# hideki1217/rusTfhe

Measured on AMD Instinct MI355X. Metric: HomNAND gates/sec (whole node), N=1024, higher is better.
Workload: dtype f64

## Files before the change

rustfhe_amd/csrc/rtfhe_context.hip:

```cpp
#include "rtfhe_host.hpp"

#include <cmath>
#include <cstdio>
#include <cstdlib>
#include <map>
#include <mutex>

using namespace rtfhe;
using namespace rtfhe_host;

namespace {

thread_local std::string g_last_error;

std::mutex g_lds_mutex;
std::map<std::pair<int, const void*>, size_t> g_lds_granted;

int ensure_pinned(rtfhe_ctx* ctx, int slot, size_t bytes) {
    if (ctx->cap_pin[slot] >= bytes && ctx->h_pin[slot]) return 0;
    if (ctx->h_pin[slot]) HIPCHECK(ctx, hipHostFree(ctx->h_pin[slot]));
    ctx->h_pin[slot] = nullptr; ctx->cap_pin[slot] = 0;
    HIPCHECK(ctx, hipHostMalloc(&ctx->h_pin[slot], bytes ? bytes : 16, hipHostMallocDefault));
    ctx->cap_pin[slot] = bytes;
    return 0;
// ... 303 lines not shown
    if (ctx->d_a) (void)hipFree(ctx->d_a);
    if (ctx->d_b) (void)hipFree(ctx->d_b);
    if (ctx->d_c) (void)hipFree(ctx->d_c);
    for (void* h : ctx->h_pin) if (h) (void)hipHostFree(h);
    for (auto& kv : ctx->mux) for (void* m : kv.second.m) if (m) (void)hipFree(m);
    for (void* m : ctx->mux_retired) (void)hipFree(m);
    for (hipEvent_t e : ctx->ks_events) (void)hipEventDestroy(e);
    if (ctx->ev0) (void)hipEventDestroy(ctx->ev0);
    if (ctx->ev1) (void)hipEventDestroy(ctx->ev1);
    if (ctx->ev_shard) (void)hipEventDestroy(ctx->ev_shard);
    for (hipEvent_t e : ctx->ev_sh) if (e) (void)hipEventDestroy(e);
    if (ctx->stream) (void)hipStreamDestroy(ctx->stream);
    delete ctx;
}

int rtfhe_set_backend(rtfhe_ctx* ctx, int backend) {
    if (int rc = use(ctx)) return rc;
    if (backend != RTFHE_BACKEND_FFT64_MIRROR && backend != RTFHE_BACKEND_NTT_EXACT && backend != RTFHE_BACKEND_FFT_SPLIT_EXACT)
        return fail(ctx, RTFHE_ERR_INVALID, "unknown backend");
    ctx->backend = backend;
    for (rtfhe_ctx* peer : ctx->peers) peer->backend = backend;
    return 0;
}

int rtfhe_get_backend(const rtfhe_ctx* ctx) { return ctx ? ctx->backend : RTFHE_ERR_INVALID; }

int rtfhe_ctx_params(const rtfhe_ctx* ctx, rtfhe_params* p) {
    if (!ctx || !p) return fail(nullptr, RTFHE_ERR_INVALID, "null argument");
    *p = ctx->p;
    return 0;
}

int rtfhe_get_twiddles(const rtfhe_ctx* ctx, double* ifft_table, double* fft_table) {
    if (!ctx || !ifft_table || !fft_table) return fail(nullptr, RTFHE_ERR_INVALID, "null argument");
    ctx->tw.export_ref(ifft_table, fft_table);
    return 0;
}

int rtfhe_set_twiddles(rtfhe_ctx* ctx, const double* ifft_table, const double* fft_table) {
    if (int rc = use(ctx)) return rc;
    if (!ifft_table || !fft_table) return fail(ctx, RTFHE_ERR_INVALID, "null argument");
    const HostTw before = ctx->tw;
    ctx->tw.import_ref(ifft_table, fft_table);
    HIPCHECK(ctx, hipDeviceSynchronize());
    if (int rc = upload_twiddles(ctx)) { ctx->tw = before; return rc; }
    if (ctx->has_bk && ctx->d_bk_torus) {
        if (int rc = transform_bk_from_torus(ctx)) return rc;
        key_changed(ctx);
        if (int rc = rebuild_derived_keys(ctx)) return rc;
    }
    for (rtfhe_ctx* peer : ctx->peers) {
        if (int rc = rtfhe_set_twiddles(peer, ifft_table, fft_table)) return fail(ctx, rc, peer->err);
        HIPCHECK(ctx, hipSetDevice(ctx->device));
    }
    return 0;
}

int rtfhe_twiddles_write(const rtfhe_ctx* ctx, const char* path) {
    if (!ctx || !path) return fail(nullptr, RTFHE_ERR_INVALID, "null argument");
    std::vector<double> t((size_t)4 * ctx->p.N);
    ctx->tw.export_ref(t.data(), t.data() + (size_t)2 * ctx->p.N);
    return rtfhe_twiddles_file_write(path, ctx->p.N, t.data(), t.data() + (size_t)2 * ctx->p.N);
}

int rtfhe_twiddles_load(rtfhe_ctx* ctx, const char* path, int32_t* entries_changed) {
    if (!ctx || !path) return fail(nullptr, RTFHE_ERR_INVALID, "null argument");
    if (entries_changed) *entries_changed = 0;
    const size_t n2 = (size_t)2 * ctx->p.N;
    std::vector<double> t(2 * n2), cur(2 * n2);
    if (rtfhe_twiddles_file_read(path, ctx->p.N, t.data(), t.data() + n2) != 0)
        return fail(ctx, RTFHE_ERR_INVALID, "twiddle table file: unreadable, wrong degree or checksum mismatch");
    ctx->tw.export_ref(cur.data(), cur.data() + n2);
    int32_t diff = 0;
    for (size_t i = 0; i < t.size(); i++) diff += std::memcmp(&t[i], &cur[i], sizeof(double)) != 0;
    if (entries_changed) *entries_changed = diff;
    if (diff == 0) return 0;
    return rtfhe_set_twiddles(ctx, t.data(), t.data() + n2);
}

int rtfhe_load_bk_torus(rtfhe_ctx* ctx, const uint32_t* bk) {
    if (int rc = use(ctx)) return rc;
    if (!bk) return fail(ctx, RTFHE_ERR_INVALID, "null argument");
    const size_t words = bk_word_count(ctx->p);
    if (!ctx->d_bk) HIPCHECK(ctx, hipMalloc((void**)&ctx->d_bk, bk_cplx_count(ctx->p) * sizeof(cplx)));
    if (!ctx->d_bk_torus) HIPCHECK(ctx, hipMalloc((void**)&ctx->d_bk_torus, words * 4));
    HIPCHECK(ctx, hipMemcpy(ctx->d_bk_torus, bk, words * 4, hipMemcpyHostToDevice));
    if (int rc = transform_bk_from_torus(ctx)) return rc;
    key_changed(ctx);
    ctx->has_bk = true;
    if (int rc = rebuild_derived_keys(ctx)) return rc;
    for (rtfhe_ctx* peer : ctx->peers) {
        if (int rc = replicate(ctx, peer, ctx->d_bk, (void**)&peer->d_bk, bk_cplx_count(ctx->p) * sizeof(cplx))) return rc;
        if (int rc = replicate(ctx, peer, ctx->d_bk_torus, (void**)&peer->d_bk_torus, words * 4)) return rc;
        key_changed(peer); peer->has_bk = true;
        if (int rc = rebuild_derived_keys(peer)) return fail(ctx, rc, peer->err);
    }
    HIPCHECK(ctx, hipSetDevice(ctx->device));
    return 0;
}

int rtfhe_load_bk_fft(rtfhe_ctx* ctx, const double* bk_f) {
    if (int rc = use(ctx)) return rc;
    if (!bk_f) return fail(ctx, RTFHE_ERR_INVALID, "null argument");
    const size_t words = bk_word_count(ctx->p);
    if (!ctx->d_bk) HIPCHECK(ctx, hipMalloc((void**)&ctx->d_bk, bk_cplx_count(ctx->p) * sizeof(cplx)));
    if (int rc = ensure(ctx, &ctx->d_a, &ctx->cap_a, words * 8)) return rc;
    HIPCHECK(ctx, hipMemcpy(ctx->d_a, bk_f, words * 8, hipMemcpyHostToDevice));
    const size_t polys = words / ctx->p.N;
    if (int rc = launch_bk_permute(ctx, (const double*)ctx->d_a, (double*)ctx->d_bk, polys, 0, ctx->stream)) return rc;
    HIPCHECK(ctx, hipStreamSynchronize(ctx->stream));
    if (ctx->d_bk_torus) { (void)hipFree(ctx->d_bk_torus); ctx->d_bk_torus = nullptr; }
    key_changed(ctx);
    ctx->has_bk = true;
    if (int rc = rebuild_derived_keys(ctx)) return rc;
    for (rtfhe_ctx* peer : ctx->peers) {
        if (int rc = replicate(ctx, peer, ctx->d_bk, (void**)&peer->d_bk, bk_cplx_count(ctx->p) * sizeof(cplx))) return rc;
        if (peer->d_bk_torus) { (void)hipSetDevice(peer->device); (void)hipFree(peer->d_bk_torus); peer->d_bk_torus = nullptr; (void)hipSetDevice(ctx->device); }
        key_changed(peer); peer->has_bk = true;
        if (int rc = rebuild_derived_keys(peer)) return fail(ctx, rc, peer->err);
    }
    HIPCHECK(ctx, hipSetDevice(ctx->device));
    return 0;
}

int rtfhe_export_bk_fft(rtfhe_ctx* ctx, double* bk_f) {
    if (int rc = use(ctx)) return rc;
    if (!bk_f) return fail(ctx, RTFHE_ERR_INVALID, "null argument");
    if (!ctx->has_bk) return fail(ctx, RTFHE_ERR_STATE, "bootstrapping key not loaded");
    const size_t words = bk_word_count(ctx->p);
    if (int rc = ensure(ctx, &ctx->d_a, &ctx->cap_a, words * 8)) return rc;
    const size_t polys = words / ctx->p.N;
    if (int rc = launch_bk_permute(ctx, (const double*)ctx->d_bk, (double*)ctx->d_a, polys, 1, ctx->stream)) return rc;
    HIPCHECK(ctx, hipStreamSynchronize(ctx->stream));
    HIPCHECK(ctx, hipMemcpy(bk_f, ctx->d_a, words * 8, hipMemcpyDeviceToHost));
    return 0;
}

int rtfhe_load_ksk(rtfhe_ctx* ctx, const uint32_t* ksk) {
    if (int rc = use(ctx)) return rc;
    if (!ksk) return fail(ctx, RTFHE_ERR_INVALID, "null argument");
    const size_t rows = ksk_rows(ctx->p), w = (size_t)ctx->p.n + 1, ksw = (size_t)ctx->ksw;
    std::vector<uint32_t> padded((rows + 1) * ksw, 0u);
    for (size_t r = 0; r < rows; r++) std::memcpy(padded.data() + r * ksw, ksk + r * w, w * 4);
    if (int rc = ensure(ctx, &ctx->d_a, &ctx->cap_a, padded.size() * 4)) return rc;
    HIPCHECK(ctx, hipMemcpy(ctx->d_a, padded.data(), padded.size() * 4, hipMemcpyHostToDevice));
    const size_t dev_rows = (size_t)ks_dev_rows(ctx->p.N, ctx->p.ks_t, ctx->p.ks_basebit);
    ctx->ksk_bytes = (dev_rows + 1) * ksw * 4;
    if (!ctx->d_ksk) HIPCHECK(ctx, hipMalloc((void**)&ctx->d_ksk, ctx->ksk_bytes));
    if (int rc = launch_ksk_combine(ctx, (const uint32_t*)ctx->d_a, ctx->stream)) return rc;
    HIPCHECK(ctx, hipStreamSynchronize(ctx->stream));
    size_t ksmat_bytes = 0;
    if (ctx->ks_mm_min > 0) {
        const int colgroups = (ctx->p.n + 1 + 15) / 16;
        ksmat_bytes = (size_t)colgroups * (ctx->p.N / 2) * 4 * 64 * sizeof(uint4);
        if (!ctx->d_ksmat) HIPCHECK(ctx, hipMalloc((void**)&ctx->d_ksmat, ksmat_bytes));
        ctx->ksmat_bytes = ksmat_bytes;
        if (int rc = launch_ksmat_build(ctx, (const uint32_t*)ctx->d_a, colgroups, ctx->stream)) return rc;
        HIPCHECK(ctx, hipStreamSynchronize(ctx->stream));
        if (int rc = ensure_tlwe1(ctx, ctx->tlwe1[ctx->stream], 8192)) return rc;
    }
    ctx->has_ksk = true;
    for (rtfhe_ctx* peer : ctx->peers) {
        if (int rc = replicate(ctx, peer, ctx->d_ksk, (void**)&peer->d_ksk, ctx->ksk_bytes)) return rc;
        peer->ksk_bytes = ctx->ksk_bytes;
        if (ksmat_bytes) {
            if (int rc = replicate(ctx, peer, ctx->d_ksmat, (void**)&peer->d_ksmat, ksmat_bytes)) return rc;
            peer->ksmat_bytes = ksmat_bytes;
        }
        peer->has_ksk = true;
    }
    return 0;
}

int rtfhe_load_ksk_ref(rtfhe_ctx* ctx, const uint32_t* ksk_ref) {
    if (int rc = use(ctx)) return rc;
    if (!ksk_ref) return fail(ctx, RTFHE_ERR_INVALID, "null argument");
    const size_t w = (size_t)ctx->p.n + 1, base = (size_t)1 << ctx->p.ks_basebit, levels = (size_t)ctx->p.N * ctx->p.ks_t;
    std::vector<uint32_t> compact;
    try { compact.resize(levels * (base - 1) * w); } catch (const std::bad_alloc&) { return fail(ctx, RTFHE_ERR_NOMEM, "host staging for the key-switching key"); }
    for (size_t il = 0; il < levels; il++)
        std::memcpy(compact.data() + il * (base - 1) * w, ksk_ref + il * base * w, (base - 1) * w * sizeof(uint32_t));
    return rtfhe_load_ksk(ctx, compact.data());
}

}
```

rustfhe_amd/csrc/rtfhe_kernels_ksmm.hpp:

```cpp
#pragma once

#include "rtfhe_kernels.hpp"

namespace rtfhe {

struct KsMmArgs {
    const uint32_t* tlwe1;
    const uint4* kmat;
    uint32_t* out;
    int32_t count, n, N, colgroups;
    int32_t splitk;
    int32_t mgroups;
    const int32_t* ops; const int32_t* idx0; const int32_t* idx1; const int32_t* idx_out;
    int32_t num_wires;
};

typedef int v4i_t __attribute__((ext_vector_type(4)));

constexpr int KSMM_WAVES = 8;
constexpr int KSMM_CHUNK = 4;
template <int KS_T, int KS_BB>
__global__ __launch_bounds__(64 * KSMM_WAVES, 1) void k_key_switch_mm(const KsMmArgs a) {
    static_assert(KS_T == 8 && KS_BB == 2, "operand packing: 4 levels x 4 digit values per 16-byte operand chunk");
    constexpr int MT = 4, W = KSMM_WAVES, KC = KSMM_CHUNK, NT = 64 * W;
    constexpr int CHUNK_V4 = KC * 4 * 64;
    constexpr int PER_THREAD = CHUNK_V4 / NT;
    static_assert(CHUNK_V4 % NT == 0, "whole uint4 per thread");
    constexpr uint32_t ROUND = 1u << (32 - KS_T * KS_BB - 1);
    const int tid = threadIdx.x, lane = tid & 63, r16 = lane & 15, q = lane >> 4;
    const int wave = __builtin_amdgcn_readfirstlane(tid >> 6);
    const int cg8 = (a.colgroups + 7) >> 3, rest = blockIdx.x >> 3, panel = rest / a.mgroups;
    const int cg = (panel % cg8) * 8 + (blockIdx.x & 7), slice = panel / cg8;
    if (cg >= a.colgroups) return;
    const int mg = (rest % a.mgroups) * W + wave;
    const int quarter = a.N / 4, ksteps = a.N / 2;
    const int kk_begin = quarter / a.splitk * slice, kk_end = kk_begin + quarter / a.splitk;
    __shared__ v4i_t onehot[256];
    __shared__ v4i_t kbuf[2][CHUNK_V4];
    for (int b = tid; b < 256; b += NT)
        onehot[b] = (v4i_t){(int)(1u << (((b >> 6) & 3) * 8)), (int)(1u << (((b >> 4) & 3) * 8)), (int)(1u << (((b >> 2) & 3) * 8)), (int)(1u << ((b & 3) * 8))};
    v4i_t acc[MT][4];
#pragma unroll
    for (int mt = 0; mt < MT; mt++)
#pragma unroll
        for (int j = 0; j < 4; j++) acc[mt][j] = (v4i_t){0, 0, 0, 0};
    const int ntiles = (a.count + 15) >> 4, tile_bytes = (int)(ext_tile_words(a.N) * 4);
    const __amdgpu_buffer_rsrc_t srsrc = __builtin_amdgcn_make_buffer_rsrc(const_cast<uint32_t*>(a.tlwe1), 0, ntiles * tile_bytes, 0x00020000);
    int tile_soff[MT];
#pragma unroll
    for (int mt = 0; mt < MT; mt++) tile_soff[mt] = __builtin_amdgcn_readfirstlane(min(mg * MT + mt, ntiles - 1) * tile_bytes);
    const int lane16 = lane * 16;
    typedef unsigned int v4u __attribute__((ext_vector_type(4)));
    const __amdgpu_buffer_rsrc_t krsrc = __builtin_amdgcn_make_buffer_rsrc(const_cast<uint4*>(a.kmat + (size_t)cg * ksteps * 4 * 64), 0, 0x7fffffff, 0x00020000);
    const int tid16 = tid * 16;
    v4u stage[PER_THREAD];
    auto fetch_chunk = [&](int ks0) {
        const int soff = __builtin_amdgcn_readfirstlane(ks0 * 4096);
#pragma unroll
        for (int p = 0; p < PER_THREAD; p++) stage[p] = __builtin_amdgcn_raw_buffer_load_b128(krsrc, tid16 + p * NT * 16, soff, 0);
    };
    auto store_chunk = [&](int buf) {
#pragma unroll
        for (int p = 0; p < PER_THREAD; p++) kbuf[buf][tid + p * NT] = (v4i_t){(int)stage[p].x, (int)stage[p].y, (int)stage[p].z, (int)stage[p].w};
    };
    const int nchunks = (kk_end - kk_begin) * 2 / KC;
    fetch_chunk(2 * kk_begin);
    store_chunk(0);
    __syncthreads();
    uint4 aw[MT];
#pragma unroll 1
    for (int c = 0; c < nchunks; c++) {
        const int kk2 = kk_begin + c * (KC / 2);
        if (c + 1 < nchunks) fetch_chunk(2 * kk2 + KC);
        if ((c & 1) == 0) {
#pragma unroll
            for (int mt = 0; mt < MT; mt++) {
                const v4u w = __builtin_amdgcn_raw_buffer_load_b128(srsrc, lane16, tile_soff[mt] + __builtin_amdgcn_readfirstlane(kk2 * 256), 0);
                aw[mt] = make_uint4(w.x, w.y, w.z, w.w);
            }
        }
        const v4i_t* kb = kbuf[c & 1] + lane;
#pragma unroll
        for (int t = 0; t < KC; t++) {
            const int h = t & 1;
            v4i_t b[4];
#pragma unroll
            for (int j = 0; j < 4; j++) b[j] = kb[(t * 4 + j) * 64];
#pragma unroll
            for (int mt = 0; mt < MT; mt++) {
                const uint32_t w0 = (c & 1) ? ((t >> 1) ? aw[mt].w : aw[mt].z) : ((t >> 1) ? aw[mt].y : aw[mt].x);
                const uint32_t byte8 = ((w0 + ROUND) >> (24 - 8 * h)) & 0xffu;
                const v4i_t av = onehot[byte8];
#pragma unroll
                for (int j = 0; j < 4; j++) acc[mt][j] = __builtin_amdgcn_mfma_i32_16x16x64_i8(av, b[j], acc[mt][j], 0, 0, 0);
            }
        }
        if (c + 1 < nchunks) store_chunk((c + 1) & 1);
        __syncthreads();
    }
    const int col = cg * 16 + r16;
    if (col > a.n) return;
#pragma unroll
    for (int mt = 0; mt < MT; mt++) {
#pragma unroll
        for (int r = 0; r < 4; r++) {
            const int g = (mg * MT + mt) * 16 + 4 * q + r;
            if (g >= a.count) continue;
            size_t row = (size_t)g;
            if (a.idx_out) {
                const int i0 = a.idx0[g], i1 = a.idx1[g], o = a.idx_out[g];
                const unsigned nw = (unsigned)a.num_wires;
                if (!((unsigned)i0 < nw && (unsigned)i1 < nw && (unsigned)o < nw && (unsigned)a.ops[g] <= (unsigned)OP_ANDNY)) continue;
                row = (size_t)o;
            }
            const uint32_t s = (uint32_t)acc[mt][0][r] + ((uint32_t)acc[mt][1][r] << 8) + ((uint32_t)acc[mt][2][r] << 16) + ((uint32_t)acc[mt][3][r] << 24);
            const uint32_t bprime = (col == a.n && slice == 0) ? a.tlwe1[(size_t)(g >> 4) * ext_tile_words(a.N) + 16 * a.N + (g & 15)] : 0u;
            atomicAdd(a.out + row * ((size_t)a.n + 1) + col, bprime - s);
        }
    }
}

struct KsMatArgs {
    const uint32_t* raw;
    uint4* kmat;
    int32_t N, n, ksw, colgroups;
};
template <int KS_T, int KS_BB>
__global__ __launch_bounds__(256) void k_ksmat_build(const KsMatArgs a) {
    const int ksteps = a.N / 2, quarter = a.N / 4;
    const size_t total = (size_t)a.colgroups * ksteps * 4 * 64;
    for (size_t idx = (size_t)blockIdx.x * blockDim.x + threadIdx.x; idx < total; idx += (size_t)gridDim.x * blockDim.x) {
        const int lane = (int)(idx & 63), limb = (int)((idx >> 6) & 3);
        const size_t rest = idx >> 8;
        const int ks = (int)(rest % ksteps), cg = (int)(rest / ksteps);
        const int col = cg * 16 + (lane & 15), q = lane >> 4, kk = ks >> 1, h = ks & 1, i = q * quarter + kk;
        uint32_t out[4] = {0, 0, 0, 0};
        if (col <= a.n) {
            for (int t = 0; t < 16; t++) {
                const int l = 4 * h + (t >> 2), d = t & 3;
                if (d == 0) continue;
                uint32_t w = a.raw[((size_t)(i * KS_T + l) * ((1 << KS_BB) - 1) + (d - 1)) * a.ksw + col];
                int32_t s = 0;
                for (int j = 0; j <= limb; j++) {
                    s = (int32_t)(int8_t)(w & 0xffu);
                    w = (w - (uint32_t)s) >> 8;
                }
                out[t >> 2] |= ((uint32_t)s & 0xffu) << (8 * (t & 3));
            }
        }
        a.kmat[idx] = make_uint4(out[0], out[1], out[2], out[3]);
    }
}

}
```

rustfhe_amd/csrc/rtfhe_stages.hip:

```cpp
#include "rtfhe_host.hpp"
#include <cmath>

#include "rtfhe_kernels_ksmm.hpp"
#include "rtfhe_kernels_anyn.hpp"

using namespace rtfhe;
using namespace rtfhe_host;

namespace {

template <int LOGN>
int launch_fft_t(rtfhe_ctx* ctx, bool forward, FftArgs a, hipStream_t s) {
    constexpr int W = 4;
    typedef Geo<LOGN> G;
    const size_t lds = (size_t)G::TW_DIR * sizeof(cplx) + (size_t)W * G::XSLOTS * sizeof(double);
    int grid = (a.count + W - 1) / W;
    if (grid > 2048) grid = 2048;
    if (forward) {
        auto k = k_fft_forward<LOGN, W>;
        if (int rc = allow_lds(ctx, k, lds)) return rc;
        hipLaunchKernelGGL(k, dim3(grid), dim3(64 * W), lds, s, a);
    } else {
        auto k = k_fft_inverse<LOGN, W>;
        if (int rc = allow_lds(ctx, k, lds)) return rc;
        hipLaunchKernelGGL(k, dim3(grid), dim3(64 * W), lds, s, a);
    }
    HIPCHECK(ctx, hipGetLastError());
    return 0;
}
template <int LOGN>
int launch_extprod_t(rtfhe_ctx* ctx, ExtProdArgs a, hipStream_t s) {
    constexpr int W = 4;
    auto k = k_external_product<LOGN, 3, 6, W>;
    const size_t lds = bootstrap_lds_bytes<LOGN>(W, 0);
    if (int rc = allow_lds(ctx, k, lds)) return rc;
    hipLaunchKernelGGL(k, dim3((a.count + W - 1) / W), dim3(64 * W), lds, s, a);
    HIPCHECK(ctx, hipGetLastError());
    return 0;
}

template <int LOGN>
int launch_keyswitch_t(rtfhe_ctx* ctx, KeySwitchArgs a, hipStream_t s) {
    constexpr int W = 4;
    auto k = k_key_switch<LOGN, 8, 2, KSQ, W>;
    const size_t lds = (size_t)W * (1 << LOGN) * 4;
    hipLaunchKernelGGL(k, dim3((a.count + W - 1) / W), dim3(64 * W), lds, s, a);
    HIPCHECK(ctx, hipGetLastError());
    return 0;
}

template <int LOGN>
int launch_keyswitch_ext_t(rtfhe_ctx* ctx, KeySwitchExtArgs a, hipStream_t s) {
    constexpr int W = 4;
    auto k = k_key_switch_ext<LOGN, 8, 2, KSQ, W>;
    const size_t lds = (size_t)W * (1 << LOGN) * 4;
    hipLaunchKernelGGL(k, dim3((a.count + W - 1) / W), dim3(64 * W), lds, s, a);
    HIPCHECK(ctx, hipGetLastError());
    ctx->launches++;
    return 0;
}

template <int LOGN>
int launch_permute_t(rtfhe_ctx* ctx, const double* src, double* dst, size_t count, int dir, int rows, hipStream_t s) {
    hipLaunchKernelGGL(k_bk_permute<LOGN>, dim3(2048), dim3(256), 0, s, src, dst, count, dir, rows);
    HIPCHECK(ctx, hipGetLastError());
    return 0;
}

template <int LOGN>
int launch_poly_mul_t(rtfhe_ctx* ctx, PolyMulArgs a, hipStream_t s) {
    constexpr int W = 4;
    typedef Geo<LOGN> G;
    auto k = k_poly_mul<LOGN, W>;
    const size_t lds = (size_t)G::TW_TOTAL * sizeof(cplx) + (size_t)W * G::XSLOTS * sizeof(double);
    if (int rc = allow_lds(ctx, k, lds)) return rc;
    int grid = (a.count + W - 1) / W;
    if (grid > 2048) grid = 2048;
    hipLaunchKernelGGL(k, dim3(grid), dim3(64 * W), lds, s, a);
    HIPCHECK(ctx, hipGetLastError());
    return 0;
}

}

namespace rtfhe_host {

int launch_fft(rtfhe_ctx* ctx, bool forward, FftArgs a, hipStream_t s) {
    if (a.count == 0) return 0;
    return ctx->logn == 10 ? launch_fft_t<10>(ctx, forward, a, s) : launch_fft_t<11>(ctx, forward, a, s);
}

int launch_bk_permute(rtfhe_ctx* ctx, const double* src, double* dst, size_t polys, int dir, hipStream_t s) {
    return ctx->logn == 10 ? launch_permute_t<10>(ctx, src, dst, polys, dir, 2 * ctx->p.l, s) : launch_permute_t<11>(ctx, src, dst, polys, dir, 2 * ctx->p.l, s);
}

int launch_ksk_combine(rtfhe_ctx* ctx, const uint32_t* d_raw, hipStream_t s) {
    KskCombineArgs a{d_raw, ctx->d_ksk, ctx->p.N, ctx->ksw};
    hipLaunchKernelGGL((k_ksk_combine<8, 2>), dim3(4096), dim3(256), 0, s, a);
    HIPCHECK(ctx, hipGetLastError());
    return 0;
}

int launch_ksmat_build(rtfhe_ctx* ctx, const uint32_t* d_raw, int colgroups, hipStream_t s) {
    KsMatArgs m{d_raw, ctx->d_ksmat, ctx->p.N, ctx->p.n, ctx->ksw, colgroups};
    hipLaunchKernelGGL((k_ksmat_build<8, 2>), dim3(4096), dim3(256), 0, s, m);
    HIPCHECK(ctx, hipGetLastError());
    return 0;
}

int launch_key_switch_mm(rtfhe_ctx* ctx, const BootstrapArgs& a, const uint32_t* samples, hipStream_t s) {
    const int per_block = 16 * KSMM_MT * KSMM_WAVES;
    const int colgroups = (ctx->p.n + 1 + 15) / 16, mgroups = (a.count + per_block - 1) / per_block;
    int splitk = 1;
    {
        double best = 0;
        for (int sk = 1; sk <= 32 && (ctx->p.N / 4) % (4 * sk) == 0; sk *= 2) {
            const double rounds = (double)mgroups * colgroups * sk / ctx->num_cus;
            const double eff = rounds / std::ceil(rounds) * std::min(1.0, rounds / 2.0);
            if (eff > best + 0.03) { best = eff; splitk = sk; }
        }
    }
    hipEvent_t ev_a = nullptr, ev_b = nullptr;
    if (ctx->timing && !ctx->tlwe1_capture && ctx->ks_events_used + 2 <= 8192) {
        while (ctx->ks_events.size() < ctx->ks_events_used + 2) { hipEvent_t e; HIPCHECK(ctx, hipEventCreate(&e)); ctx->ks_events.push_back(e); }
        ev_a = ctx->ks_events[ctx->ks_events_used]; ev_b = ctx->ks_events[ctx->ks_events_used + 1];
        ctx->ks_events_used += 2;
        HIPCHECK(ctx, hipEventRecord(ev_a, s));
    }
    const size_t w1 = (size_t)ctx->p.N + 1, seg_max = ((size_t)1 << 31) / (w1 * 4) / per_block * per_block;
    for (size_t off = 0; off < (size_t)a.count; off += seg_max) {
        const size_t cnt = std::min(seg_max, (size_t)a.count - off);
        const int mg = (int)((cnt + per_block - 1) / per_block);
        KsMmArgs k{samples + off * w1, ctx->d_ksmat, a.idx_out ? a.out : a.out + off * ((size_t)ctx->p.n + 1), (int32_t)cnt, ctx->p.n, ctx->p.N, colgroups, splitk, mg,
                   a.ops ? a.ops + off : nullptr, a.idx0 ? a.idx0 + off : nullptr, a.idx1 ? a.idx1 + off : nullptr, a.idx_out ? a.idx_out + off : nullptr, a.num_wires};
        hipLaunchKernelGGL((k_key_switch_mm<8, 2>), dim3(mg * ((colgroups + 7) / 8 * 8) * splitk), dim3(64 * KSMM_WAVES), 0, s, k);
        HIPCHECK(ctx, hipGetLastError());
    }
    if (ev_b) HIPCHECK(ctx, hipEventRecord(ev_b, s));
    ctx->launches++;
    return 0;
}

int launch_key_switch_ext(rtfhe_ctx* ctx, uint32_t* samples, uint32_t* d_out, size_t count, hipStream_t s) {
    const KeySwitchExtArgs a{ctx->d_ksk, samples, d_out, (int32_t)count, ctx->p.n, ctx->ksw};
    return ctx->logn == 10 ? launch_keyswitch_ext_t<10>(ctx, a, s) : launch_keyswitch_ext_t<11>(ctx, a, s);
}

}

extern "C" {

int rtfhe_external_product_batch(rtfhe_ctx* ctx, const int32_t* bk_index, const uint32_t* trlwe, uint32_t* out, size_t count) {
    if (int rc = use(ctx)) return rc;
    if (!bk_index || !trlwe || !out) return fail(ctx, RTFHE_ERR_INVALID, "null argument");
    if (!ctx->has_bk) return fail(ctx, RTFHE_ERR_STATE, "bootstrapping key not loaded");
    if (count == 0) return 0;
    if (count > 0x7fffffff) return fail(ctx, RTFHE_ERR_INVALID, "count too large");
    for (size_t g = 0; g < count; g++)
        if (bk_index[g] < 0 || bk_index[g] >= ctx->p.n) return fail(ctx, RTFHE_ERR_INVALID, "bk_index out of range");
    const size_t bytes = count * 2 * (size_t)ctx->p.N * 4;
    if (int rc = ensure(ctx, &ctx->d_a, &ctx->cap_a, bytes)) return rc;
    if (int rc = ensure(ctx, &ctx->d_b, &ctx->cap_b, count * 4)) return rc;
    if (int rc = ensure(ctx, &ctx->d_c, &ctx->cap_c, bytes)) return rc;
    HIPCHECK(ctx, hipMemcpyAsync(ctx->d_a, trlwe, bytes, hipMemcpyHostToDevice, ctx->stream));
    HIPCHECK(ctx, hipMemcpyAsync(ctx->d_b, bk_index, count * 4, hipMemcpyHostToDevice, ctx->stream));
    int rc;
    if (ctx->backend == RTFHE_BACKEND_NTT_EXACT) {
        if ((rc = ntt_prepare(ctx))) return rc;
        if ((rc = launch_extprod_ntt(ctx, (const int32_t*)ctx->d_b, (const uint32_t*)ctx->d_a, (uint32_t*)ctx->d_c, (int32_t)count, ctx->stream))) return rc;
    } else if (ctx->backend == RTFHE_BACKEND_FFT_SPLIT_EXACT) {
        if ((rc = xfft_prepare(ctx))) return rc;
        if ((rc = launch_extprod_xfft(ctx, (const int32_t*)ctx->d_b, (const uint32_t*)ctx->d_a, (uint32_t*)ctx->d_c, (int32_t)count, ctx->stream))) return rc;
    } else {
        ExtProdArgs a{ctx->d_tw, ctx->d_bk, (const int32_t*)ctx->d_b, (const uint32_t*)ctx->d_a, (uint32_t*)ctx->d_c, (int32_t)count};
        rc = ctx->logn == 10 ? launch_extprod_t<10>(ctx, a, ctx->stream) : launch_extprod_t<11>(ctx, a, ctx->stream);
        if (rc) return rc;
    }
    HIPCHECK(ctx, hipMemcpyAsync(out, ctx->d_c, bytes, hipMemcpyDeviceToHost, ctx->stream));
    HIPCHECK(ctx, hipStreamSynchronize(ctx->stream));
    return 0;
}

int rtfhe_key_switch_batch(rtfhe_ctx* ctx, const uint32_t* tlwe1, uint32_t* out, size_t count) {
    if (int rc = use(ctx)) return rc;
    if (!tlwe1 || !out) return fail(ctx, RTFHE_ERR_INVALID, "null argument");
    if (!ctx->has_ksk) return fail(ctx, RTFHE_ERR_STATE, "key-switching key not loaded");
    if (count == 0) return 0;
    if (count > 0x7fffffff) return fail(ctx, RTFHE_ERR_INVALID, "count too large");
    const size_t in_bytes = count * ((size_t)ctx->p.N + 1) * 4, out_bytes = count * ((size_t)ctx->p.n + 1) * 4;
    if (int rc = ensure(ctx, &ctx->d_a, &ctx->cap_a, in_bytes)) return rc;
    if (int rc = ensure(ctx, &ctx->d_c, &ctx->cap_c, out_bytes)) return rc;
    HIPCHECK(ctx, hipMemcpyAsync(ctx->d_a, tlwe1, in_bytes, hipMemcpyHostToDevice, ctx->stream));
    KeySwitchArgs a{ctx->d_ksk, (const uint32_t*)ctx->d_a, (uint32_t*)ctx->d_c, (int32_t)count, ctx->p.n, ctx->ksw};
    int rc = ctx->logn == 10 ? launch_keyswitch_t<10>(ctx, a, ctx->stream) : launch_keyswitch_t<11>(ctx, a, ctx->stream);
    if (rc) return rc;
    HIPCHECK(ctx, hipMemcpyAsync(out, ctx->d_c, out_bytes, hipMemcpyDeviceToHost, ctx->stream));
    HIPCHECK(ctx, hipStreamSynchronize(ctx->stream));
    return 0;
}

static int run_fft_batch(rtfhe_ctx* ctx, bool forward, bool f64_io, const void* src, void* res, size_t count) {
    if (int rc = use(ctx)) return rc;
    if (!src || !res) return fail(ctx, RTFHE_ERR_INVALID, "null argument");
    if (count == 0) return 0;
    if (count > 0x7fffffff) return fail(ctx, RTFHE_ERR_INVALID, "count too large");
    const size_t N = (size_t)ctx->p.N;
    const size_t in_bytes = count * N * ((forward && !f64_io) ? 4 : 8), out_bytes = count * N * ((forward || f64_io) ? 8 : 4);
    if (int rc = ensure(ctx, &ctx->d_a, &ctx->cap_a, in_bytes)) return rc;
    if (int rc = ensure(ctx, &ctx->d_c, &ctx->cap_c, out_bytes)) return rc;
    HIPCHECK(ctx, hipMemcpyAsync(ctx->d_a, src, in_bytes, hipMemcpyHostToDevice, ctx->stream));
    FftArgs a{ctx->d_tw, ctx->d_a, ctx->d_c, (int32_t)count, 0, 0, f64_io ? 1 : 0};
    if (int rc = launch_fft(ctx, forward, a, ctx->stream)) return rc;
    HIPCHECK(ctx, hipMemcpyAsync(res, ctx->d_c, out_bytes, hipMemcpyDeviceToHost, ctx->stream));
    HIPCHECK(ctx, hipStreamSynchronize(ctx->stream));
    return 0;
}

int rtfhe_ifft_i32_batch(rtfhe_ctx* ctx, const int32_t* src, double* res, size_t count) {
    return run_fft_batch(ctx, true, false, src, res, count);
}

int rtfhe_fft_u32_batch(rtfhe_ctx* ctx, const double* src, uint32_t* res, size_t count) {
    return run_fft_batch(ctx, false, false, src, res, count);
}

int rtfhe_ifft_f64_batch(rtfhe_ctx* ctx, const double* src, double* res, size_t count) {
    return run_fft_batch(ctx, true, true, src, res, count);
}

int rtfhe_fft_f64_batch(rtfhe_ctx* ctx, const double* src, double* res, size_t count) {
    return run_fft_batch(ctx, false, true, src, res, count);
}

int rtfhe_poly_mul_batch(rtfhe_ctx* ctx, const uint32_t* a, const uint32_t* b, uint32_t* res, size_t count) {
    if (int rc = use(ctx)) return rc;
    if (!a || !b || !res) return fail(ctx, RTFHE_ERR_INVALID, "null argument");
    if (count == 0) return 0;
    if (count > 0x7fffffff) return fail(ctx, RTFHE_ERR_INVALID, "count too large");
    const size_t bytes = count * (size_t)ctx->p.N * 4;
    if (int rc = ensure(ctx, &ctx->d_a, &ctx->cap_a, bytes)) return rc;
    if (int rc = ensure(ctx, &ctx->d_b, &ctx->cap_b, bytes)) return rc;
    if (int rc = ensure(ctx, &ctx->d_c, &ctx->cap_c, bytes)) return rc;
    HIPCHECK(ctx, hipMemcpyAsync(ctx->d_a, a, bytes, hipMemcpyHostToDevice, ctx->stream));
    HIPCHECK(ctx, hipMemcpyAsync(ctx->d_b, b, bytes, hipMemcpyHostToDevice, ctx->stream));
    PolyMulArgs pa{ctx->d_tw, (const uint32_t*)ctx->d_a, (const uint32_t*)ctx->d_b, (uint32_t*)ctx->d_c, (int32_t)count};
    int rc = ctx->logn == 10 ? launch_poly_mul_t<10>(ctx, pa, ctx->stream) : launch_poly_mul_t<11>(ctx, pa, ctx->stream);
    if (rc) return rc;
    HIPCHECK(ctx, hipMemcpyAsync(res, ctx->d_c, bytes, hipMemcpyDeviceToHost, ctx->stream));
    HIPCHECK(ctx, hipStreamSynchronize(ctx->stream));
    return 0;
}

}

struct rtfhe_fft_plan {
    int32_t N = 0;
    int device = 0;
    HostTw tw;
    double* d_tab = nullptr;
    void* d_in = nullptr; void* d_in2 = nullptr; void* d_out = nullptr;
    size_t cap = 0;
    hipStream_t stream = nullptr;
};

namespace {

#define PLANCHECK(expr)                                                                              \
    do {                                                                                             \
        hipError_t e__ = (expr);                                                                     \
        if (e__ != hipSuccess)                                                                       \
            return fail(nullptr, RTFHE_ERR_HIP, std::string(#expr) + ": " + hipGetErrorString(e__)); \
    } while (0)

int plan_upload(rtfhe_fft_plan* pl) {
    const int P = pl->N / 2;
    std::vector<double> t((size_t)8 * P);
    const std::vector<double>* src[8] = {&pl->tw.twist_c, &pl->tw.twist_s, &pl->tw.untw_c, &pl->tw.untw_s,
                                         &pl->tw.fwd_c, &pl->tw.fwd_s, &pl->tw.inv_c, &pl->tw.inv_s};
    for (int k = 0; k < 8; k++) std::memcpy(t.data() + (size_t)k * P, src[k]->data(), sizeof(double) * P);
    PLANCHECK(hipMemcpy(pl->d_tab, t.data(), t.size() * sizeof(double), hipMemcpyHostToDevice));
    return 0;
}

int plan_run(rtfhe_fft_plan* pl, int mode, const void* src, const void* src2, void* res, size_t count) {
    if (!pl) return fail(nullptr, RTFHE_ERR_INVALID, "null plan");
    if (!src || !res || (mode == ANYN_POLY_MUL && !src2)) return fail(nullptr, RTFHE_ERR_INVALID, "null argument");
    if (count == 0) return 0;
    if (count > 0x7fffffff) return fail(nullptr, RTFHE_ERR_INVALID, "count too large");
    PLANCHECK(hipSetDevice(pl->device));
    const size_t N = (size_t)pl->N;
    if (pl->cap < count) {
        for (void** b : {&pl->d_in, &pl->d_in2, &pl->d_out}) { if (*b) PLANCHECK(hipFree(*b)); *b = nullptr; }
        pl->cap = 0;
        for (void** b : {&pl->d_in, &pl->d_in2, &pl->d_out}) PLANCHECK(hipMalloc(b, count * N * 8));
        pl->cap = count;
    }
    const size_t in_bytes = count * N * ((mode == ANYN_IFFT_I32 || mode == ANYN_POLY_MUL) ? 4 : 8);
    const size_t out_bytes = count * N * ((mode == ANYN_FFT_U32 || mode == ANYN_POLY_MUL) ? 4 : 8);
    PLANCHECK(hipMemcpyAsync(pl->d_in, src, in_bytes, hipMemcpyHostToDevice, pl->stream));
    if (mode == ANYN_POLY_MUL) PLANCHECK(hipMemcpyAsync(pl->d_in2, src2, in_bytes, hipMemcpyHostToDevice, pl->stream));
    AnyNArgs a{pl->d_tab, pl->d_in, pl->d_in2, pl->d_out, pl->N, (int32_t)count, mode};
    const unsigned grid = (unsigned)(count < 4096 ? count : 4096);
    hipLaunchKernelGGL(k_fft_anyn, dim3(grid), dim3(ANYN_THREADS), 0, pl->stream, a);
    PLANCHECK(hipGetLastError());
    PLANCHECK(hipMemcpyAsync(res, pl->d_out, out_bytes, hipMemcpyDeviceToHost, pl->stream));
    PLANCHECK(hipStreamSynchronize(pl->stream));
    return 0;
}

}

extern "C" {

int rtfhe_fft_plan_create(int32_t N, int device_id, rtfhe_fft_plan** out) {
    if (!out) return fail(nullptr, RTFHE_ERR_INVALID, "null argument");
    *out = nullptr;
    if (N < 16 || N > 2 * ANYN_MAXP || (N & (N - 1))) return fail(nullptr, RTFHE_ERR_INVALID, "supported transform sizes: powers of two 16 <= N <= 2048");
    int ndev = 0;
    if (hipGetDeviceCount(&ndev) != hipSuccess || ndev <= 0)
        return fail(nullptr, RTFHE_ERR_NO_DEVICE, "no HIP device available (this library has no CPU fallback)");
    if (device_id < 0 || device_id >= ndev) return fail(nullptr, RTFHE_ERR_INVALID, "device_id out of range");
    rtfhe_fft_plan* pl = new (std::nothrow) rtfhe_fft_plan();
    if (!pl) return fail(nullptr, RTFHE_ERR_NOMEM, "out of host memory");
    pl->N = N; pl->device = device_id;
    pl->tw.build(N);
    int rc = 0;
    if (hipSetDevice(device_id) != hipSuccess || hipMalloc((void**)&pl->d_tab, (size_t)8 * (N / 2) * sizeof(double)) != hipSuccess ||
        hipStreamCreate(&pl->stream) != hipSuccess)
        rc = fail(nullptr, RTFHE_ERR_HIP, "device set-up of the transform plan failed");
    if (!rc) rc = plan_upload(pl);
    if (rc) { rtfhe_fft_plan_destroy(pl); return rc; }
    *out = pl;
    return 0;
}

void rtfhe_fft_plan_destroy(rtfhe_fft_plan* pl) {
    if (!pl) return;
    (void)hipSetDevice(pl->device);
    if (pl->stream) { (void)hipStreamSynchronize(pl->stream); (void)hipStreamDestroy(pl->stream); }
    for (void* b : {(void*)pl->d_tab, pl->d_in, pl->d_in2, pl->d_out}) if (b) (void)hipFree(b);
    delete pl;
}

int32_t rtfhe_fft_plan_degree(const rtfhe_fft_plan* pl) { return pl ? pl->N : 0; }

int rtfhe_fft_plan_get_twiddles(const rtfhe_fft_plan* pl, double* ifft_table, double* fft_table) {
    if (!pl || !ifft_table || !fft_table) return fail(nullptr, RTFHE_ERR_INVALID, "null argument");
    pl->tw.export_ref(ifft_table, fft_table);
// ... 20 lines not shown
```

Baseline: 158,100.

## Pack three nonzero key-switch digits per MFMA operand and use persistent team scheduling

The key-switch matrix encoding drops the always-zero digit value, packing 4 levels x 3 nonzero digits into 12-byte units. This cuts the K dimension of the int8 MFMA GEMM from N/2 to 3N/8 steps, and with it the key-matrix bytes streamed. The split-K grid is replaced by a persistent team/member schedule that sizes work to resident workgroups (two per CU via waves_per_eu) and loops over column-group segments with prefetch across segments. The standalone key_switch_batch API is also routed through the MFMA path via a new tile-conversion kernel, which adds complexity and more LDS per workgroup.

```diff
diff --git a/rustfhe_amd/csrc/rtfhe_context.hip b/rustfhe_amd/csrc/rtfhe_context.hip
--- a/rustfhe_amd/csrc/rtfhe_context.hip
+++ b/rustfhe_amd/csrc/rtfhe_context.hip
@@ -479,7 +479,7 @@
     size_t ksmat_bytes = 0;
     if (ctx->ks_mm_min > 0) {
         const int colgroups = (ctx->p.n + 1 + 15) / 16;
-        ksmat_bytes = (size_t)colgroups * (ctx->p.N / 2) * 4 * 64 * sizeof(uint4);
+        ksmat_bytes = (size_t)colgroups * (ctx->p.N / 8 * 3) * 4 * 64 * sizeof(uint4);
         if (!ctx->d_ksmat) HIPCHECK(ctx, hipMalloc((void**)&ctx->d_ksmat, ksmat_bytes));
         ctx->ksmat_bytes = ksmat_bytes;
         if (int rc = launch_ksmat_build(ctx, (const uint32_t*)ctx->d_a, colgroups, ctx->stream)) return rc;
diff --git a/rustfhe_amd/csrc/rtfhe_kernels_ksmm.hpp b/rustfhe_amd/csrc/rtfhe_kernels_ksmm.hpp
--- a/rustfhe_amd/csrc/rtfhe_kernels_ksmm.hpp
+++ b/rustfhe_amd/csrc/rtfhe_kernels_ksmm.hpp
@@ -9,8 +9,9 @@
     const uint4* kmat;
     uint32_t* out;
     int32_t count, n, N, colgroups;
-    int32_t splitk;
     int32_t mgroups;
+    int32_t members;
+    int32_t span;
     const int32_t* ops; const int32_t* idx0; const int32_t* idx1; const int32_t* idx_out;
     int32_t num_wires;
 };
@@ -18,104 +19,134 @@
 typedef int v4i_t __attribute__((ext_vector_type(4)));
 
 constexpr int KSMM_WAVES = 8;
-constexpr int KSMM_CHUNK = 4;
+constexpr int KSMM_CHUNK = 3;
+constexpr int KSMM_WGS_PER_CU = 2;
 template <int KS_T, int KS_BB>
-__global__ __launch_bounds__(64 * KSMM_WAVES, 1) void k_key_switch_mm(const KsMmArgs a) {
-    static_assert(KS_T == 8 && KS_BB == 2, "operand packing: 4 levels x 4 digit values per 16-byte operand chunk");
+__global__ __launch_bounds__(64 * KSMM_WAVES) __attribute__((amdgpu_waves_per_eu(4, 4))) void k_key_switch_mm(const KsMmArgs a) {
+    static_assert(KS_T == 8 && KS_BB == 2, "operand packing: 4 levels x 3 non-zero digit values per 12-byte unit");
     constexpr int MT = 4, W = KSMM_WAVES, KC = KSMM_CHUNK, NT = 64 * W;
     constexpr int CHUNK_V4 = KC * 4 * 64;
-    constexpr int PER_THREAD = CHUNK_V4 / NT;
-    static_assert(CHUNK_V4 % NT == 0, "whole uint4 per thread");
+    constexpr int PER_THREAD = (CHUNK_V4 + NT - 1) / NT;
+    static_assert(CHUNK_V4 % NT % 64 == 0, "whole waves stage the last round");
+    static_assert(KSMM_WGS_PER_CU * ((256 + 2 * CHUNK_V4) * sizeof(v4i_t) + MT * 2 * NT * 4) <= 160 * 1024, "the table, both chunk buffers and the digit bytes of every resident workgroup fit a CU's LDS");
     constexpr uint32_t ROUND = 1u << (32 - KS_T * KS_BB - 1);
     const int tid = threadIdx.x, lane = tid & 63, r16 = lane & 15, q = lane >> 4;
     const int wave = __builtin_amdgcn_readfirstlane(tid >> 6);
-    const int cg8 = (a.colgroups + 7) >> 3, rest = blockIdx.x >> 3, panel = rest / a.mgroups;
-    const int cg = (panel % cg8) * 8 + (blockIdx.x & 7), slice = panel / cg8;
-    if (cg >= a.colgroups) return;
-    const int mg = (rest % a.mgroups) * W + wave;
-    const int quarter = a.N / 4, ksteps = a.N / 2;
-    const int kk_begin = quarter / a.splitk * slice, kk_end = kk_begin + quarter / a.splitk;
+    const int xcd = blockIdx.x & 7, rank = blockIdx.x >> 3, team = rank / a.members, member = rank % a.members;
+    const int cpc = a.N / 16, ksteps = a.N / 8 * 3;
+    const int ncg = xcd < a.colgroups ? (a.colgroups - 1 - xcd) / 8 + 1 : 0;
+    const int u_begin = team * a.span, u_end = min(u_begin + a.span, ncg * cpc);
+    if (u_begin >= u_end) return;
     __shared__ v4i_t onehot[256];
     __shared__ v4i_t kbuf[2][CHUNK_V4];
-    for (int b = tid; b < 256; b += NT)
-        onehot[b] = (v4i_t){(int)(1u << (((b >> 6) & 3) * 8)), (int)(1u << (((b >> 4) & 3) * 8)), (int)(1u << (((b >> 2) & 3) * 8)), (int)(1u << ((b & 3) * 8))};
+    __shared__ uint32_t awbuf[MT][2][NT];
+    for (int b = tid; b < 256; b += NT) {
+        uint32_t w[3] = {0u, 0u, 0u};
+#pragma unroll
+        for (int j = 0; j < 4; j++) {
+            const int d = (b >> (6 - 2 * j)) & 3, pos = 3 * j + d - 1;
+            if (d) w[pos >> 2] |= 1u << (8 * (pos & 3));
+        }
+        onehot[b] = (v4i_t){(int)w[0], (int)w[1], (int)w[2], 0};
+    }
+    const uint32_t* onehot_w = reinterpret_cast<const uint32_t*>(onehot);
     v4i_t acc[MT][4];
-#pragma unroll
-    for (int mt = 0; mt < MT; mt++)
-#pragma unroll
-        for (int j = 0; j < 4; j++) acc[mt][j] = (v4i_t){0, 0, 0, 0};
     const int ntiles = (a.count + 15) >> 4, tile_bytes = (int)(ext_tile_words(a.N) * 4);
     const __amdgpu_buffer_rsrc_t srsrc = __builtin_amdgcn_make_buffer_rsrc(const_cast<uint32_t*>(a.tlwe1), 0, ntiles * tile_bytes, 0x00020000);
-    int tile_soff[MT];
-#pragma unroll
-    for (int mt = 0; mt < MT; mt++) tile_soff[mt] = __builtin_amdgcn_readfirstlane(min(mg * MT + mt, ntiles - 1) * tile_bytes);
     const int lane16 = lane * 16;
     typedef unsigned int v4u __attribute__((ext_vector_type(4)));
-    const __amdgpu_buffer_rsrc_t krsrc = __builtin_amdgcn_make_buffer_rsrc(const_cast<uint4*>(a.kmat + (size_t)cg * ksteps * 4 * 64), 0, 0x7fffffff, 0x00020000);
     const int tid16 = tid * 16;
     v4u stage[PER_THREAD];
-    auto fetch_chunk = [&](int ks0) {
-        const int soff = __builtin_amdgcn_readfirstlane(ks0 * 4096);
+    auto fetch_chunk = [&](int cg, int hc) {
+        const __amdgpu_buffer_rsrc_t krsrc = __builtin_amdgcn_make_buffer_rsrc(const_cast<uint4*>(a.kmat + (size_t)cg * ksteps * 4 * 64), 0, ksteps * 4096, 0x00020000);
+        const int soff = __builtin_amdgcn_readfirstlane(hc * (KC * 4096));
 #pragma unroll
-        for (int p = 0; p < PER_THREAD; p++) stage[p] = __builtin_amdgcn_raw_buffer_load_b128(krsrc, tid16 + p * NT * 16, soff, 0);
+        for (int p = 0; p < PER_THREAD; p++)
+            if (tid + p * NT < CHUNK_V4) stage[p] = __builtin_amdgcn_raw_buffer_load_b128(krsrc, tid16 + p * NT * 16, soff, 0);
     };
     auto store_chunk = [&](int buf) {
 #pragma unroll
-        for (int p = 0; p < PER_THREAD; p++) kbuf[buf][tid + p * NT] = (v4i_t){(int)stage[p].x, (int)stage[p].y, (int)stage[p].z, (int)stage[p].w};
+        for (int p = 0; p < PER_THREAD; p++)
+            if (tid + p * NT < CHUNK_V4) kbuf[buf][tid + p * NT] = (v4i_t){(int)stage[p].x, (int)stage[p].y, (int)stage[p].z, (int)stage[p].w};
     };
-    const int nchunks = (kk_end - kk_begin) * 2 / KC;
-    fetch_chunk(2 * kk_begin);
+    const int i_first = u_begin / cpc, i_last = (u_end - 1) / cpc, per_pass = i_last - i_first + 1;
+    const int nseg = ((a.mgroups - member + a.members - 1) / a.members) * per_pass;
+    fetch_chunk(i_first * 8 + xcd, 2 * (u_begin - i_first * cpc));
     store_chunk(0);
     __syncthreads();
-    uint4 aw[MT];
 #pragma unroll 1
-    for (int c = 0; c < nchunks; c++) {
-        const int kk2 = kk_begin + c * (KC / 2);
-        if (c + 1 < nchunks) fetch_chunk(2 * kk2 + KC);
-        if ((c & 1) == 0) {
+    for (int seg = 0; seg < nseg; seg++) {
+        const int i = i_first + seg % per_pass, cg = i * 8 + xcd, mgb = member + seg / per_pass * a.members;
+        const int ch0 = max(u_begin - i * cpc, 0), ch1 = min(u_end - i * cpc, cpc);
+        const int mg = mgb * W + wave;
+        int tile_soff[MT];
+#pragma unroll
+        for (int mt = 0; mt < MT; mt++) tile_soff[mt] = __builtin_amdgcn_readfirstlane(min(mg * MT + mt, ntiles - 1) * tile_bytes);
+#pragma unroll
+        for (int mt = 0; mt < MT; mt++)
+#pragma unroll
+            for (int j = 0; j < 4; j++) acc[mt][j] = (v4i_t){0, 0, 0, 0};
+#pragma unroll 1
+        for (int hc = 2 * ch0; hc < 2 * ch1; hc++) {
+            const int pr = hc & 1;
+            if (hc + 1 < 2 * ch1) fetch_chunk(cg, hc + 1);
+            if (pr == 0) {
+#pragma unroll
+                for (int mt = 0; mt < MT; mt++) {
+                    const v4u w = __builtin_amdgcn_raw_buffer_load_b128(srsrc, lane16, tile_soff[mt] + __builtin_amdgcn_readfirstlane(hc * 512), 0) + ROUND;
+                    awbuf[mt][0][tid] = (w.x >> 16) | (w.y & 0xffff0000u);
+                    awbuf[mt][1][tid] = (w.z >> 16) | (w.w & 0xffff0000u);
+                }
+            }
+            const v4i_t* kb = kbuf[pr] + lane;
+#pragma unroll
+            for (int s = 0; s < KC; s++) {
+                v4i_t b[4];
+#pragma unroll
+                for (int j = 0; j < 4; j++) b[j] = kb[(s * 4 + j) * 64];
+#pragma unroll
+                for (int mt = 0; mt < MT; mt++) {
+                    const uint32_t e = awbuf[mt][pr][tid];
+                    const uint32_t us = s == 0 ? (e >> 8) & 0xffu : s == 1 ? e & 0xffu : e >> 24;
+                    const uint32_t u3 = (e >> 16) & 0xffu;
+                    v4i_t av = onehot[us];
+                    av.w = (int)onehot_w[u3 * 4 + s];
+#pragma unroll
+                    for (int j = 0; j < 4; j++) acc[mt][j] = __builtin_amdgcn_mfma_i32_16x16x64_i8(av, b[j], acc[mt][j], 0, 0, 0);
+                }
+            }
+            if (hc + 1 < 2 * ch1) store_chunk(pr ^ 1);
+            __syncthreads();
+        }
+        const bool more = seg + 1 < nseg;
+        if (more) {
+            const int i2 = i_first + (seg + 1) % per_pass;
+            fetch_chunk(i2 * 8 + xcd, 2 * max(u_begin - i2 * cpc, 0));
+        }
+        const int col = cg * 16 + r16;
+        if (col <= a.n) {
 #pragma unroll
             for (int mt = 0; mt < MT; mt++) {
-                const v4u w = __builtin_amdgcn_raw_buffer_load_b128(srsrc, lane16, tile_soff[mt] + __builtin_amdgcn_readfirstlane(kk2 * 256), 0);
-                aw[mt] = make_uint4(w.x, w.y, w.z, w.w);
+#pragma unroll
+                for (int r = 0; r < 4; r++) {
+                    const int g = (mg * MT + mt) * 16 + 4 * q + r;
+                    if (g >= a.count) continue;
+                    size_t row = (size_t)g;
+                    if (a.idx_out) {
+                        const int i0 = a.idx0[g], i1 = a.idx1[g], o = a.idx_out[g];
+                        const unsigned nw = (unsigned)a.num_wires;
+                        if (!((unsigned)i0 < nw && (unsigned)i1 < nw && (unsigned)o < nw && (unsigned)a.ops[g] <= (unsigned)OP_ANDNY)) continue;
+                        row = (size_t)o;
+                    }
+                    const uint32_t s = (uint32_t)acc[mt][0][r] + ((uint32_t)acc[mt][1][r] << 8) + ((uint32_t)acc[mt][2][r] << 16) + ((uint32_t)acc[mt][3][r] << 24);
+                    const uint32_t bprime = (col == a.n && ch0 == 0) ? a.tlwe1[(size_t)(g >> 4) * ext_tile_words(a.N) + 16 * a.N + (g & 15)] : 0u;
+                    atomicAdd(a.out + row * ((size_t)a.n + 1) + col, bprime - s);
+                }
             }
         }
-        const v4i_t* kb = kbuf[c & 1] + lane;
-#pragma unroll
-        for (int t = 0; t < KC; t++) {
-            const int h = t & 1;
-            v4i_t b[4];
-#pragma unroll
-            for (int j = 0; j < 4; j++) b[j] = kb[(t * 4 + j) * 64];
-#pragma unroll
-            for (int mt = 0; mt < MT; mt++) {
-                const uint32_t w0 = (c & 1) ? ((t >> 1) ? aw[mt].w : aw[mt].z) : ((t >> 1) ? aw[mt].y : aw[mt].x);
-                const uint32_t byte8 = ((w0 + ROUND) >> (24 - 8 * h)) & 0xffu;
-                const v4i_t av = onehot[byte8];
-#pragma unroll
-                for (int j = 0; j < 4; j++) acc[mt][j] = __builtin_amdgcn_mfma_i32_16x16x64_i8(av, b[j], acc[mt][j], 0, 0, 0);
-            }
-        }
-        if (c + 1 < nchunks) store_chunk((c + 1) & 1);
-        __syncthreads();
-    }
-    const int col = cg * 16 + r16;
-    if (col > a.n) return;
-#pragma unroll
-    for (int mt = 0; mt < MT; mt++) {
-#pragma unroll
-        for (int r = 0; r < 4; r++) {
-            const int g = (mg * MT + mt) * 16 + 4 * q + r;
-            if (g >= a.count) continue;
-            size_t row = (size_t)g;
-            if (a.idx_out) {
-                const int i0 = a.idx0[g], i1 = a.idx1[g], o = a.idx_out[g];
-                const unsigned nw = (unsigned)a.num_wires;
-                if (!((unsigned)i0 < nw && (unsigned)i1 < nw && (unsigned)o < nw && (unsigned)a.ops[g] <= (unsigned)OP_ANDNY)) continue;
-                row = (size_t)o;
-            }
-            const uint32_t s = (uint32_t)acc[mt][0][r] + ((uint32_t)acc[mt][1][r] << 8) + ((uint32_t)acc[mt][2][r] << 16) + ((uint32_t)acc[mt][3][r] << 24);
-            const uint32_t bprime = (col == a.n && slice == 0) ? a.tlwe1[(size_t)(g >> 4) * ext_tile_words(a.N) + 16 * a.N + (g & 15)] : 0u;
-            atomicAdd(a.out + row * ((size_t)a.n + 1) + col, bprime - s);
+        if (more) {
+            store_chunk(0);
+            __syncthreads();
         }
     }
 }
@@ -127,29 +158,40 @@
 };
 template <int KS_T, int KS_BB>
 __global__ __launch_bounds__(256) void k_ksmat_build(const KsMatArgs a) {
-    const int ksteps = a.N / 2, quarter = a.N / 4;
+    const int ksteps = a.N / 8 * 3, quarter = a.N / 4;
     const size_t total = (size_t)a.colgroups * ksteps * 4 * 64;
     for (size_t idx = (size_t)blockIdx.x * blockDim.x + threadIdx.x; idx < total; idx += (size_t)gridDim.x * blockDim.x) {
         const int lane = (int)(idx & 63), limb = (int)((idx >> 6) & 3);
         const size_t rest = idx >> 8;
         const int ks = (int)(rest % ksteps), cg = (int)(rest / ksteps);
-        const int col = cg * 16 + (lane & 15), q = lane >> 4, kk = ks >> 1, h = ks & 1, i = q * quarter + kk;
+        const int col = cg * 16 + (lane & 15), q = lane >> 4, p = ks / 3, s = ks % 3, e = q * quarter + 2 * p;
         uint32_t out[4] = {0, 0, 0, 0};
         if (col <= a.n) {
             for (int t = 0; t < 16; t++) {
-                const int l = 4 * h + (t >> 2), d = t & 3;
-                if (d == 0) continue;
+                const int i = t < 12 ? e + (s >> 1) : e + 1, h = t < 12 ? (s & 1) : 1, pos = t < 12 ? t : 4 * s + t - 12;
+                const int l = 4 * h + pos / 3, d = pos % 3 + 1;
                 uint32_t w = a.raw[((size_t)(i * KS_T + l) * ((1 << KS_BB) - 1) + (d - 1)) * a.ksw + col];
-                int32_t s = 0;
+                int32_t sb = 0;
                 for (int j = 0; j <= limb; j++) {
-                    s = (int32_t)(int8_t)(w & 0xffu);
-                    w = (w - (uint32_t)s) >> 8;
+                    sb = (int32_t)(int8_t)(w & 0xffu);
+                    w = (w - (uint32_t)sb) >> 8;
                 }
-                out[t >> 2] |= ((uint32_t)s & 0xffu) << (8 * (t & 3));
+                out[t >> 2] |= ((uint32_t)sb & 0xffu) << (8 * (t & 3));
             }
         }
         a.kmat[idx] = make_uint4(out[0], out[1], out[2], out[3]);
     }
 }
 
+struct ExtTileArgs {
+    const uint32_t* rows;
+    uint32_t* ext;
+    int32_t count, N;
+};
+__global__ __launch_bounds__(256) void k_ext_tile(const ExtTileArgs a) {
+    const size_t w1 = (size_t)a.N + 1, total = (size_t)a.count * w1;
+    for (size_t idx = (size_t)blockIdx.x * blockDim.x + threadIdx.x; idx < total; idx += (size_t)gridDim.x * blockDim.x)
+        *ext_slot(a.ext, (int)(idx / w1), (int)(idx % w1), a.N) = a.rows[idx];
 }
+
+}
diff --git a/rustfhe_amd/csrc/rtfhe_stages.hip b/rustfhe_amd/csrc/rtfhe_stages.hip
--- a/rustfhe_amd/csrc/rtfhe_stages.hip
+++ b/rustfhe_amd/csrc/rtfhe_stages.hip
@@ -1,4 +1,5 @@
 #include "rtfhe_host.hpp"
+#include <algorithm>
 #include <cmath>
 
 #include "rtfhe_kernels_ksmm.hpp"
@@ -111,15 +112,9 @@
 int launch_key_switch_mm(rtfhe_ctx* ctx, const BootstrapArgs& a, const uint32_t* samples, hipStream_t s) {
     const int per_block = 16 * KSMM_MT * KSMM_WAVES;
     const int colgroups = (ctx->p.n + 1 + 15) / 16, mgroups = (a.count + per_block - 1) / per_block;
-    int splitk = 1;
-    {
-        double best = 0;
-        for (int sk = 1; sk <= 32 && (ctx->p.N / 4) % (4 * sk) == 0; sk *= 2) {
-            const double rounds = (double)mgroups * colgroups * sk / ctx->num_cus;
-            const double eff = rounds / std::ceil(rounds) * std::min(1.0, rounds / 2.0);
-            if (eff > best + 0.03) { best = eff; splitk = sk; }
-        }
-    }
+    const int resident = std::max(1, ctx->num_cus * KSMM_WGS_PER_CU / 8), cg8 = (colgroups + 7) / 8, units = cg8 * (ctx->p.N / 16);
+    const int members = std::min(mgroups, resident);
+    const int span = std::max((units + resident / members - 1) / (resident / members), 2), teams = (units + span - 1) / span;
     hipEvent_t ev_a = nullptr, ev_b = nullptr;
     if (ctx->timing && !ctx->tlwe1_capture && ctx->ks_events_used + 2 <= 8192) {
         while (ctx->ks_events.size() < ctx->ks_events_used + 2) { hipEvent_t e; HIPCHECK(ctx, hipEventCreate(&e)); ctx->ks_events.push_back(e); }
@@ -131,9 +126,9 @@
     for (size_t off = 0; off < (size_t)a.count; off += seg_max) {
         const size_t cnt = std::min(seg_max, (size_t)a.count - off);
         const int mg = (int)((cnt + per_block - 1) / per_block);
-        KsMmArgs k{samples + off * w1, ctx->d_ksmat, a.idx_out ? a.out : a.out + off * ((size_t)ctx->p.n + 1), (int32_t)cnt, ctx->p.n, ctx->p.N, colgroups, splitk, mg,
+        KsMmArgs k{samples + off * w1, ctx->d_ksmat, a.idx_out ? a.out : a.out + off * ((size_t)ctx->p.n + 1), (int32_t)cnt, ctx->p.n, ctx->p.N, colgroups, mg, std::min(mg, members), span,
                    a.ops ? a.ops + off : nullptr, a.idx0 ? a.idx0 + off : nullptr, a.idx1 ? a.idx1 + off : nullptr, a.idx_out ? a.idx_out + off : nullptr, a.num_wires};
-        hipLaunchKernelGGL((k_key_switch_mm<8, 2>), dim3(mg * ((colgroups + 7) / 8 * 8) * splitk), dim3(64 * KSMM_WAVES), 0, s, k);
+        hipLaunchKernelGGL((k_key_switch_mm<8, 2>), dim3(8 * teams * std::min(mg, members)), dim3(64 * KSMM_WAVES), 0, s, k);
         HIPCHECK(ctx, hipGetLastError());
     }
     if (ev_b) HIPCHECK(ctx, hipEventRecord(ev_b, s));
@@ -191,9 +186,21 @@
     if (int rc = ensure(ctx, &ctx->d_a, &ctx->cap_a, in_bytes)) return rc;
     if (int rc = ensure(ctx, &ctx->d_c, &ctx->cap_c, out_bytes)) return rc;
     HIPCHECK(ctx, hipMemcpyAsync(ctx->d_a, tlwe1, in_bytes, hipMemcpyHostToDevice, ctx->stream));
-    KeySwitchArgs a{ctx->d_ksk, (const uint32_t*)ctx->d_a, (uint32_t*)ctx->d_c, (int32_t)count, ctx->p.n, ctx->ksw};
-    int rc = ctx->logn == 10 ? launch_keyswitch_t<10>(ctx, a, ctx->stream) : launch_keyswitch_t<11>(ctx, a, ctx->stream);
-    if (rc) return rc;
+    if (ctx->d_ksmat && ctx->ks_mm_min > 0) {
+        rtfhe_ctx::Tlwe1& buf = ctx->tlwe1[ctx->stream];
+        if (int rc = ensure_tlwe1(ctx, buf, count)) return rc;
+        const ExtTileArgs t{(const uint32_t*)ctx->d_a, buf.d, (int32_t)count, ctx->p.N};
+        hipLaunchKernelGGL(k_ext_tile, dim3((unsigned)std::min<size_t>((count * ((size_t)ctx->p.N + 1) + 255) / 256, 4096)), dim3(256), 0, ctx->stream, t);
+        HIPCHECK(ctx, hipGetLastError());
+        HIPCHECK(ctx, hipMemsetAsync(ctx->d_c, 0, out_bytes, ctx->stream));
+        BootstrapArgs k{};
+        k.out = (uint32_t*)ctx->d_c; k.count = (int32_t)count; k.n = ctx->p.n;
+        if (int rc = launch_key_switch_mm(ctx, k, buf.d, ctx->stream)) return rc;
+    } else {
+        KeySwitchArgs a{ctx->d_ksk, (const uint32_t*)ctx->d_a, (uint32_t*)ctx->d_c, (int32_t)count, ctx->p.n, ctx->ksw};
+        int rc = ctx->logn == 10 ? launch_keyswitch_t<10>(ctx, a, ctx->stream) : launch_keyswitch_t<11>(ctx, a, ctx->stream);
+        if (rc) return rc;
+    }
     HIPCHECK(ctx, hipMemcpyAsync(out, ctx->d_c, out_bytes, hipMemcpyDeviceToHost, ctx->stream));
     HIPCHECK(ctx, hipStreamSynchronize(ctx->stream));
     return 0;
```

Result: no change. 158,000 (-0.1%).
